# helemanc/audio-based-lyrics-matching

Hardware: NVIDIA B200
Metric: similarity+MAP eval Gpairs/s at 1/2/4/8 B200 (roofline frac); MAP parity (higher is better)
Workload: dtype f16 tensor-core hi/lo split x3, f32 accumulate

## Files before the change

audio-based-lyrics-matching_b200/csrc/eval_sym_epilogue.cuh:

```cuda
#pragma once
#include "gemm_core.cuh"

namespace wealy {

struct EvalSymParams {
  const float4* lvl;
  const uint2* cinfo;
  const int* s_c;
  const int* s_i;
  const float* thr;
  unsigned int* hist;
  const unsigned char* dirty;
  int n_col_tiles;
  int n_row_blocks;
  unsigned int total_pairs;
  const float* beta;
  float* tk_val;
  int* tk_idx;
  int* tk_cnt;
  int tk_cap;
};

__device__ __forceinline__ unsigned bit_transpose32(unsigned x, int lane) {
#pragma unroll
  for (int s = 16; s >= 1; s >>= 1) {
    const unsigned mask = s == 16 ? 0x0000ffffu : s == 8 ? 0x00ff00ffu : s == 4 ? 0x0f0f0f0fu : s == 2 ? 0x33333333u : 0x55555555u;
    const unsigned y = __shfl_xor_sync(0xffffffffu, x, s);
    x = (lane & s) ? ((x & ~mask) | ((y >> s) & mask)) : ((x & mask) | ((y << s) & ~mask));
  }
  return x;
}

template <int kLv, int kQueueCapT = 256, int kCachePairsT = 4096, bool kTopk = false>
struct EvalSymEpi {
  static_assert(kLv >= 2 && kLv <= 4, "2..4 register levels");
  static_assert(!kTopk || kLv <= 3, "the top-k bound of the columns rides in the 4th threshold slot");
  using Params = EvalSymParams;
  static constexpr int kQueueCap = kQueueCapT;
  static constexpr int kCachePairs = kCachePairsT;
  static constexpr unsigned kGlobal = 0x80000000u;
  static constexpr int kOffQx = kQueueCap * 4;
  static constexpr int kOffQn = kOffQx + kQueueCap * 4;
  static constexpr int kStageCols = 16;
  static constexpr int kOffStage = kOffQn + kQueueCap * 4;
  static constexpr int kWarpScratchBytes = kOffStage + kStageCols * 32 * 4;
  static constexpr int kColSlots = 3;
  static constexpr int kLvlBytes = kTileN * 16;
  static constexpr int kInfoBytes = kTileN * 8;
  static constexpr int kColSlotBytes = kLvlBytes + kInfoBytes;
  static constexpr int kOffColSlots = (kCachePairs * 4 + 15) / 16 * 16;
  static constexpr int kCtaScratchBytes = kOffColSlots + kColSlots * kColSlotBytes;

  __device__ static __forceinline__ void col_bulk_src(const Params& p, int t, const void*& s0, const void*& s1) {
    s0 = p.lvl + (size_t)t * kTileN;
    s1 = p.cinfo + (size_t)t * kTileN;
  }

  struct RowState {
    float t[kLv];
    unsigned rc[kLv - 1];
    unsigned rinfo;
    int rpc;
    int qc, qi;
    unsigned off;
    int qn;
    int n_cached;
    unsigned base;
    int row_glob, row_ok, dirty;
    float beta;
  };

  __device__ static __forceinline__ float* q_val(const EpiCtx& c) { return reinterpret_cast<float*>(c.warp_scratch); }
  __device__ static __forceinline__ unsigned* q_idx(const EpiCtx& c) { return reinterpret_cast<unsigned*>(c.warp_scratch + kOffQx); }
  __device__ static __forceinline__ int* q_len(const EpiCtx& c) { return reinterpret_cast<int*>(c.warp_scratch + kOffQn); }
  __device__ static __forceinline__ float* stage(const EpiCtx& c) { return reinterpret_cast<float*>(c.warp_scratch + kOffStage); }
  __device__ static __forceinline__ float* thr_s(const EpiCtx& c) { return reinterpret_cast<float*>(c.cta_scratch); }

  __device__ static __forceinline__ float lvl_of(const float4& v, int j) {
    return j == 0 ? v.x : (j == 1 ? v.y : (j == 2 ? v.z : v.w));
  }

  __device__ static __forceinline__ void row_begin(const Params& p, RowState& st, int row, int part,
                                                   const GemmShape& sh, const EpiCtx& ctx) {
    (void)part;
    const float inf = __int_as_float(0x7f800000);
#pragma unroll
    for (int j = 0; j < kLv; ++j) st.t[j] = inf;
#pragma unroll
    for (int j = 0; j < kLv - 1; ++j) st.rc[j] = 0u;
    st.qc = st.qi = 0;
    st.off = 0u;
    st.beta = inf;
    int cnt = 0;
    const int srow = spread_sorted_of(row);
    st.row_ok = srow < sh.m_rows;
    if (st.row_ok) {
      const float4 v = __ldg(p.lvl + row);
#pragma unroll
      for (int j = 0; j < kLv; ++j) st.t[j] = lvl_of(v, j);
      const uint2 ci = __ldg(p.cinfo + row);
      st.off = ci.x;
      cnt = (int)ci.y;
      st.qc = __ldg(p.s_c + srow);
      st.qi = __ldg(p.s_i + srow);
      if constexpr (kTopk) st.beta = __ldg(p.beta + row);
    }
    st.qn = 0;
    st.row_glob = row;
    st.dirty = 0;
    st.base = __ldg(p.cinfo + ctx.row_base).x;
    const unsigned end = (ctx.row_base + ctx.row_span < sh.m_rows) ? __ldg(p.cinfo + ctx.row_base + ctx.row_span).x : p.total_pairs;
    const unsigned total = end - st.base;
    st.n_cached = (int)(total < (unsigned)kCachePairs ? total : (unsigned)kCachePairs);
    float* ts = thr_s(ctx);
    for (int i = ctx.tid; i < st.n_cached; i += ctx.nthreads) ts[i] = __ldg(p.thr + st.base + i);
    const unsigned rel = st.off - st.base;
    const bool cached = st.row_ok && rel + (unsigned)cnt <= (unsigned)st.n_cached;
    st.rinfo = cached ? (rel + kLv) : (kGlobal | (st.off + kLv));
    st.rpc = cnt - kLv;
    ptx::named_barrier_sync(1, ctx.nthreads);
  }

  __device__ static __forceinline__ int warp_incl_scan(int v, int lane) {
#pragma unroll
    for (int o = 1; o < 32; o <<= 1) {
      const int t = __shfl_up_sync(0xffffffffu, v, o);
      if (lane >= o) v += t;
    }
    return v;
  }

  struct Ent {
    float s;
    unsigned idx;
    int len;
    int cand;
    bool on;
    const float* tp;
  };
  __device__ static __forceinline__ void fetch(const Params& p, const EpiCtx& ctx, Ent& en, int r, int end) {
    en.on = r < end;
    en.s = en.on ? q_val(ctx)[r] : 0.f;
    en.idx = en.on ? q_idx(ctx)[r] : 0u;
    const int raw = en.on ? q_len(ctx)[r] : 0;
    en.len = max(raw, 0);
    en.cand = kTopk ? -1 - raw : -1;
    en.tp = (en.idx & kGlobal) ? (p.thr + (en.idx & ~kGlobal)) : (thr_s(ctx) + en.idx);
  }
  __device__ static __forceinline__ void count(const Params& p, const RowState& st, const EpiCtx& ctx, const Ent& en,
                                               int lb, int lane) {
    (void)ctx; (void)lane;
    if constexpr (kTopk) {
      if (en.cand >= 0) {
        if (en.on) {
          const int pos = atomicAdd(p.tk_cnt + en.idx, 1);
          if (pos < p.tk_cap) {
            p.tk_val[(size_t)en.idx * p.tk_cap + pos] = en.s;
            p.tk_idx[(size_t)en.idx * p.tk_cap + pos] = en.cand;
          }
        }
        return;
      }
    }
    const bool glob = (en.idx & kGlobal) != 0u;
    const unsigned slot = (en.idx & ~kGlobal) - 1u + (unsigned)lb + (glob ? 0u : st.base);
    if (en.on) atomicAdd(p.hist + slot, 1u);
  }

  __device__ static __forceinline__ void drain(const Params& p, RowState& st, const EpiCtx& ctx) {
    if (st.qn == 0) return;
    const int lane = (int)ptx::lane_id();
    __syncwarp();
    const int end = st.qn;
    for (int r0 = 0; r0 < end; r0 += 64) {
      Ent a, b;
      fetch(p, ctx, a, r0 + lane, end);
      fetch(p, ctx, b, r0 + 32 + lane, end);
      int loa = 0, hia = a.len, lob = 0, hib = b.len;
      while (loa < hia || lob < hib) {
        if (loa < hia) {
          const int mid = (loa + hia) >> 1;
          if (a.tp[mid] < a.s) loa = mid + 1; else hia = mid;
        }
        if (lob < hib) {
          const int mid = (lob + hib) >> 1;
          if (b.tp[mid] < b.s) lob = mid + 1; else hib = mid;
        }
      }
      count(p, st, ctx, a, loa, lane);
      if (r0 + 32 < end) count(p, st, ctx, b, lob, lane);
    }
    __syncwarp();
    st.qn = 0;
  }

  __device__ static __forceinline__ void push(const RowState& st, const EpiCtx& ctx, const uint32_t (&acc)[32], unsigned mr,
                                              unsigned mcq, const uint2* cinf, int pos, unsigned tkr = 0u, unsigned tkc = 0u,
                                              int col0 = 0) {
    float* qv = q_val(ctx);
    unsigned* qx = q_idx(ctx);
    int* ql = q_len(ctx);
    float* stg = stage(ctx) + (ptx::lane_id());
#pragma unroll
    for (int h = 0; h < 32 / kStageCols; ++h) {
      const unsigned sel = ((1u << kStageCols) - 1u) << (h * kStageCols);
      if (!__any_sync(0xffffffffu, ((mr | mcq | tkr | tkc) & sel) != 0u)) continue;
#pragma unroll
      for (int e = 0; e < kStageCols; ++e) stg[e * 32] = __uint_as_float(acc[h * kStageCols + e]);
      unsigned m = mr & sel;
      while (m) {
        const int e = __ffs(m) - 1;
        m &= m - 1;
        qv[pos] = stg[(e - h * kStageCols) * 32];
        qx[pos] = st.rinfo;
        ql[pos] = st.rpc;
        ++pos;
      }
      m = mcq & sel;
      while (m) {
        const int e = __ffs(m) - 1;
        m &= m - 1;
        const uint2 c = cinf[e];
        qv[pos] = stg[(e - h * kStageCols) * 32];
        qx[pos] = kGlobal | (c.x + kLv);
        ql[pos] = (int)c.y - kLv;
        ++pos;
      }
      if constexpr (kTopk) {
        m = tkr & sel;
        while (m) {
          const int e = __ffs(m) - 1;
          m &= m - 1;
          qv[pos] = stg[(e - h * kStageCols) * 32];
          qx[pos] = (unsigned)st.row_glob;
          ql[pos] = -1 - (col0 + e);
          ++pos;
        }
        m = tkc & sel;
        while (m) {
          const int e = __ffs(m) - 1;
          m &= m - 1;
          qv[pos] = stg[(e - h * kStageCols) * 32];
          qx[pos] = (unsigned)(col0 + e);
          ql[pos] = -1 - st.row_glob;
          ++pos;
        }
      }
      __syncwarp();
    }
  }

  __device__ static __forceinline__ void tile_begin(const Params& p, RowState& st, const GemmShape& sh,
                                                    const EpiCtx& ctx, int t) {
    (void)sh;
    st.dirty = 0;
    for (int rbi = ctx.row_base / kTileM; rbi < (ctx.row_base + ctx.row_span) / kTileM; ++rbi)
      st.dirty |= rbi < p.n_row_blocks ? (int)__ldg(p.dirty + (size_t)rbi * p.n_col_tiles + t) : 1;
  }

  __device__ static __forceinline__ void chunk32(const Params& p, RowState& st, int row, int col0,
                                                 const uint32_t (&acc)[32], const GemmShape& sh, const EpiCtx& ctx) {
    constexpr unsigned kFull = 0xffffffffu;
    const int lane = (int)ptx::lane_id();
    (void)row;
    const float4* lv = reinterpret_cast<const float4*>(ctx.col_slot) + (col0 & (kTileN - 1));
    const uint2* cinf = reinterpret_cast<const uint2*>(ctx.col_slot + kLvlBytes) + (col0 & (kTileN - 1));

    unsigned m[kLv], mc[kLv];
    unsigned tkr = 0u, tkc = 0u;
#pragma unroll
    for (int j = 0; j < kLv; ++j) m[j] = mc[j] = 0u;
#pragma unroll
    for (int e = 0; e < 32; ++e) {
      const float s = __uint_as_float(acc[e]);
      const float4 c = lv[e];
#pragma unroll
      for (int j = 0; j < kLv; ++j) {
        m[j] |= (s > st.t[j]) ? (1u << e) : 0u;
        mc[j] |= (s > lvl_of(c, j)) ? (1u << e) : 0u;
      }
      if constexpr (kTopk) {
        tkr |= (s > st.beta) ? (1u << e) : 0u;
        tkc |= (s > c.w) ? (1u << e) : 0u;
      }
    }
    if (st.dirty) {
      const int scol = spread_sorted_of(col0 + lane);
      const bool ok = scol < sh.n_cols;
      const int cc = ok ? __ldg(p.s_c + scol) : 0;
      const int ci = ok ? __ldg(p.s_i + scol) : 0;
      unsigned valid = 0u, validk = 0u;
#pragma unroll
      for (int e = 0; e < 32; ++e) {
        const int cce = __shfl_sync(kFull, cc, e);
        const int cie = __shfl_sync(kFull, ci, e);
        const int oke = __shfl_sync(kFull, (int)ok, e);
        valid |= (oke && cce != st.qc && cie != st.qi) ? (1u << e) : 0u;
        if constexpr (kTopk) validk |= (oke && cie != st.qi) ? (1u << e) : 0u;
      }
      const int d = st.row_glob - col0;
      const unsigned above = d < 0 ? 0xffffffffu : (d >= 31 ? 0u : (0xffffffffu << (d + 1)));
      valid &= above;
      validk &= above;
      if (!st.row_ok) valid = validk = 0u;
#pragma unroll
      for (int j = 0; j < kLv; ++j) {
        m[j] &= valid;
        mc[j] &= valid;
      }
      tkr &= validk;
      tkc &= validk;
    }
    if constexpr (kTopk) {
      if (!__any_sync(kFull, (m[0] | mc[0] | tkr | tkc) != 0u)) return;
    } else {
      if (!__any_sync(kFull, (m[0] | mc[0]) != 0u)) return;
    }

#pragma unroll
    for (int j = 0; j < kLv - 1; ++j) st.rc[j] += (unsigned)__popc(m[j] ^ m[j + 1]);
    if (__any_sync(kFull, (mc[0] ^ mc[kLv - 1]) != 0u)) {
      const unsigned coff = cinf[lane].x;
#pragma unroll
      for (int j = 0; j < kLv - 1; ++j) {
        const unsigned n = (unsigned)__popc(bit_transpose32(mc[j] ^ mc[j + 1], lane));
        if (n != 0u) atomicAdd(p.hist + coff + j, n);
      }
    }

    const unsigned dr = m[kLv - 1], dc = mc[kLv - 1];
    if (!__any_sync(kFull, (dr | dc | tkr | tkc) != 0u)) return;
    const int mine = __popc(dr) + __popc(dc) + __popc(tkr) + __popc(tkc);
    const int incl = warp_incl_scan(mine, lane);
    const int total = __shfl_sync(kFull, incl, 31);
    if (st.qn + total > kQueueCap) drain(p, st, ctx);
    if (total <= kQueueCap) {
      push(st, ctx, acc, dr, dc, cinf, st.qn + incl - mine, tkr, tkc, col0);
      st.qn += total;
    } else {
      constexpr int kBatchCols = kQueueCap / (kTopk ? 128 : 64);
      static_assert(kBatchCols >= 1 && 32 % kBatchCols == 0, "queue capacity: 64 (128 with top-k) .. 2048, a power of two");
#pragma unroll 1
      for (int g = 0; g < 32 / kBatchCols; ++g) {
        const unsigned sel = ((1u << kBatchCols) - 1u) << (kBatchCols * g);
        const int mine_g = __popc(dr & sel) + __popc(dc & sel) + __popc(tkr & sel) + __popc(tkc & sel);
        const int incl_g = warp_incl_scan(mine_g, lane);
        push(st, ctx, acc, dr & sel, dc & sel, cinf, incl_g - mine_g, tkr & sel, tkc & sel, col0);
        st.qn = __shfl_sync(kFull, incl_g, 31);
        drain(p, st, ctx);
      }
    }
  }

  __device__ static __forceinline__ void tile_end(const Params& p, RowState& st, const GemmShape&, const EpiCtx& ctx) {
    if (st.qn >= kQueueCap / 2) drain(p, st, ctx);
  }

  __device__ static __forceinline__ void row_end(const Params& p, RowState& st, int row, int part,
                                                 const GemmShape& sh, const EpiCtx& ctx) {
    (void)row; (void)part; (void)sh;
    drain(p, st, ctx);
    if (st.row_ok) {
#pragma unroll
      for (int j = 0; j < kLv - 1; ++j)
        if (st.rc[j] != 0u) atomicAdd(p.hist + st.off + j, st.rc[j]);
    }
    ptx::named_barrier_sync(1, ctx.nthreads);
  }
};

}
```

audio-based-lyrics-matching_b200/csrc/ptx.cuh:

```cuda
#pragma once
#include <cstdint>
#include <cuda.h>
#include <cuda_runtime.h>

namespace wealy {
namespace ptx {

__device__ __forceinline__ uint32_t smem_u32(const void* p) {
  return static_cast<uint32_t>(__cvta_generic_to_shared(p));
}

__device__ __forceinline__ uint32_t lane_id() {
  uint32_t l;
  asm volatile("mov.u32 %0, %%laneid;" : "=r"(l));
  return l;
}

__device__ __forceinline__ void mbar_init(uint64_t* bar, uint32_t count) {
  asm volatile("mbarrier.init.shared::cta.b64 [%0], %1;" ::"r"(smem_u32(bar)), "r"(count));
}

__device__ __forceinline__ void fence_mbar_init() {
  asm volatile("fence.mbarrier_init.release.cluster;" ::: "memory");
}

__device__ __forceinline__ void fence_proxy_async() {
  asm volatile("fence.proxy.async.shared::cta;" ::: "memory");
}

__device__ __forceinline__ void mbar_expect_tx(uint64_t* bar, uint32_t bytes) {
  asm volatile("mbarrier.arrive.expect_tx.shared::cta.b64 _, [%0], %1;" ::"r"(smem_u32(bar)), "r"(bytes)
               : "memory");
}

__device__ __forceinline__ void mbar_arrive(uint64_t* bar) {
  asm volatile("mbarrier.arrive.shared::cta.b64 _, [%0];" ::"r"(smem_u32(bar)) : "memory");
}

#ifndef WEALY_WAIT_HINT_NS
#define WEALY_WAIT_HINT_NS 1000
#endif
#ifndef WEALY_WAIT_ALL_LANES
#define WEALY_WAIT_LANE0
#endif

__device__ __forceinline__ bool mbar_try_wait(uint64_t* bar, uint32_t parity) {
  uint32_t ok;
#if WEALY_WAIT_HINT_NS > 0
  asm volatile(
      "{\n"
      ".reg .pred P;\n"
      "mbarrier.try_wait.parity.shared::cta.b64 P, [%1], %2, %3;\n"
      "selp.u32 %0, 1, 0, P;\n"
      "}\n"
      : "=r"(ok)
      : "r"(smem_u32(bar)), "r"(parity), "r"((uint32_t)WEALY_WAIT_HINT_NS)
      : "memory");
#else
  asm volatile(
      "{\n"
      ".reg .pred P;\n"
      "mbarrier.try_wait.parity.shared::cta.b64 P, [%1], %2;\n"
      "selp.u32 %0, 1, 0, P;\n"
      "}\n"
      : "=r"(ok)
      : "r"(smem_u32(bar)), "r"(parity)
      : "memory");
#endif
  return ok != 0;
}

#ifndef WEALY_DEADLOCK_CYCLES
#define WEALY_DEADLOCK_CYCLES (4000000000ll)
#endif

__device__ __forceinline__ void mbar_wait(uint64_t* bar, uint32_t parity) {
  if (mbar_try_wait(bar, parity)) return;
  const long long t0 = clock64();
  int polls = 0;
  while (!mbar_try_wait(bar, parity)) {
    if ((++polls & 63) == 0 && clock64() - t0 > WEALY_DEADLOCK_CYCLES) {
      printf("wealy: mbarrier deadlock block=%d thread=%d bar=0x%x parity=%u\n", (int)blockIdx.x,
             (int)threadIdx.x, smem_u32(bar), parity);
      __trap();
    }
  }
}

__device__ __forceinline__ void mbar_wait_warp(uint64_t* bar, uint32_t parity) {
#ifdef WEALY_WAIT_LANE0
  if (lane_id() == 0) mbar_wait(bar, parity);
  __syncwarp();
#else
  mbar_wait(bar, parity);
#endif
}

__device__ __forceinline__ void named_barrier_sync(int id, int nthreads) {
  asm volatile("bar.sync %0, %1;" ::"r"(id), "r"(nthreads) : "memory");
}

__device__ __forceinline__ void prefetch_tensormap(const CUtensorMap* m) {
  asm volatile("prefetch.tensormap [%0];" ::"l"(reinterpret_cast<uint64_t>(m)) : "memory");
}

__device__ __forceinline__ void tma_load_2d(void* smem_dst, const CUtensorMap* m, uint64_t* bar, int32_t c0,
                                            int32_t c1, uint64_t cache_policy) {
  asm volatile(
      "cp.async.bulk.tensor.2d.shared::cluster.global.mbarrier::complete_tx::bytes.L2::cache_hint"
      " [%0], [%1, {%3, %4}], [%2], %5;"
      ::"r"(smem_u32(smem_dst)), "l"(reinterpret_cast<uint64_t>(m)), "r"(smem_u32(bar)), "r"(c0), "r"(c1),
        "l"(cache_policy)
      : "memory");
}

__device__ __forceinline__ void bulk_load(void* smem_dst, const void* gsrc, uint32_t bytes, uint64_t* bar) {
  asm volatile(
      "cp.async.bulk.shared::cluster.global.mbarrier::complete_tx::bytes [%0], [%1], %2, [%3];"
      ::"r"(smem_u32(smem_dst)), "l"(reinterpret_cast<uint64_t>(gsrc)), "r"(bytes), "r"(smem_u32(bar))
      : "memory");
}

constexpr uint64_t kEvictNormal = 0x1000000000000000ull;
constexpr uint64_t kEvictFirst = 0x12F0000000000000ull;
constexpr uint64_t kEvictLast = 0x14F0000000000000ull;

template <uint32_t kCols>
__device__ __forceinline__ void tmem_alloc(uint32_t* smem_result) {
  static_assert(kCols >= 32 && kCols <= 512 && (kCols & (kCols - 1)) == 0, "TMEM columns: power of two in [32,512]");
  asm volatile("tcgen05.alloc.cta_group::1.sync.aligned.shared::cta.b32 [%0], %1;" ::"r"(smem_u32(smem_result)),
               "n"(kCols)
               : "memory");
  asm volatile("tcgen05.relinquish_alloc_permit.cta_group::1.sync.aligned;" ::: "memory");
}

template <uint32_t kCols>
__device__ __forceinline__ void tmem_dealloc(uint32_t tmem_addr) {
  asm volatile("tcgen05.dealloc.cta_group::1.sync.aligned.b32 %0, %1;" ::"r"(tmem_addr), "n"(kCols) : "memory");
}

__device__ __forceinline__ void tc_fence_before_sync() {
  asm volatile("tcgen05.fence::before_thread_sync;" ::: "memory");
}
__device__ __forceinline__ void tc_fence_after_sync() {
  asm volatile("tcgen05.fence::after_thread_sync;" ::: "memory");
}

__device__ __forceinline__ void umma_f16(uint32_t tmem_d, uint64_t desc_a, uint64_t desc_b, uint32_t idesc,
                                         uint32_t accumulate) {
  asm volatile(
      "{\n"
      ".reg .pred p;\n"
      "setp.ne.b32 p, %4, 0;\n"
      "tcgen05.mma.cta_group::1.kind::f16 [%0], %1, %2, %3, p;\n"
      "}\n"
      ::"r"(tmem_d), "l"(desc_a), "l"(desc_b), "r"(idesc), "r"(accumulate)
      : "memory");
}

__device__ __forceinline__ void umma_commit(uint64_t* bar) {
  asm volatile("tcgen05.commit.cta_group::1.mbarrier::arrive::one.shared::cluster.b64 [%0];" ::"r"(smem_u32(bar))
               : "memory");
}

__device__ __forceinline__ void tmem_ld_32x32(uint32_t taddr, uint32_t (&v)[32]) {
  asm volatile(
      "tcgen05.ld.sync.aligned.32x32b.x32.b32 "
      "{%0, %1, %2, %3, %4, %5, %6, %7, %8, %9, %10, %11, %12, %13, %14, %15, "
      "%16, %17, %18, %19, %20, %21, %22, %23, %24, %25, %26, %27, %28, %29, %30, %31}, [%32];"
      : "=r"(v[0]), "=r"(v[1]), "=r"(v[2]), "=r"(v[3]), "=r"(v[4]), "=r"(v[5]), "=r"(v[6]), "=r"(v[7]), "=r"(v[8]),
        "=r"(v[9]), "=r"(v[10]), "=r"(v[11]), "=r"(v[12]), "=r"(v[13]), "=r"(v[14]), "=r"(v[15]), "=r"(v[16]),
        "=r"(v[17]), "=r"(v[18]), "=r"(v[19]), "=r"(v[20]), "=r"(v[21]), "=r"(v[22]), "=r"(v[23]), "=r"(v[24]),
        "=r"(v[25]), "=r"(v[26]), "=r"(v[27]), "=r"(v[28]), "=r"(v[29]), "=r"(v[30]), "=r"(v[31])
      : "r"(taddr)
      : "memory");
}

__device__ __forceinline__ void tmem_ld_wait() { asm volatile("tcgen05.wait::ld.sync.aligned;" ::: "memory"); }


__device__ __forceinline__ uint32_t cluster_ctarank() {
  uint32_t r;
  asm volatile("mov.u32 %0, %%cluster_ctarank;" : "=r"(r));
  return r;
}
__device__ __forceinline__ uint32_t cluster_id_x() {
  uint32_t r;
  asm volatile("mov.u32 %0, %%clusterid.x;" : "=r"(r));
  return r;
}
__device__ __forceinline__ uint32_t n_clusters_x() {
  uint32_t r;
  asm volatile("mov.u32 %0, %%nclusterid.x;" : "=r"(r));
  return r;
}
__device__ __forceinline__ void cluster_sync_all() {
  asm volatile("barrier.cluster.arrive.release.aligned;\n\tbarrier.cluster.wait.acquire.aligned;" ::: "memory");
}
__device__ __forceinline__ uint32_t map_to_cta(const void* p, uint32_t rank) {
  uint32_t r;
  asm volatile("mapa.shared::cluster.u32 %0, %1, %2;" : "=r"(r) : "r"(smem_u32(p)), "r"(rank));
  return r;
}
__device__ __forceinline__ void mbar_arrive_cluster(uint32_t cluster_addr) {
  asm volatile("mbarrier.arrive.release.cluster.shared::cluster.b64 _, [%0];" ::"r"(cluster_addr) : "memory");
}
__device__ __forceinline__ void mbar_arrive_cluster_relaxed(uint32_t cluster_addr) {
  asm volatile("mbarrier.arrive.relaxed.cluster.shared::cluster.b64 _, [%0];" ::"r"(cluster_addr) : "memory");
}
__device__ __forceinline__ void st_cluster_u32(uint32_t cluster_addr, uint32_t v) {
  asm volatile("st.shared::cluster.u32 [%0], %1;" ::"r"(cluster_addr), "r"(v) : "memory");
}
__device__ __forceinline__ void mbar_wait_cluster(uint64_t* bar, uint32_t parity) {
  const long long t0 = clock64();
  int polls = 0;
  while (true) {
    uint32_t ok;
    asm volatile(
        "{\n"
        ".reg .pred P;\n"
        "mbarrier.try_wait.parity.acquire.cluster.shared::cta.b64 P, [%1], %2, %3;\n"
        "selp.u32 %0, 1, 0, P;\n"
        "}\n"
        : "=r"(ok)
        : "r"(smem_u32(bar)), "r"(parity), "r"((uint32_t)(WEALY_WAIT_HINT_NS > 0 ? WEALY_WAIT_HINT_NS : 1))
        : "memory");
    if (ok) return;
    if ((++polls & 63) == 0 && clock64() - t0 > WEALY_DEADLOCK_CYCLES) {
      printf("wealy: cluster mbarrier deadlock block=%d thread=%d bar=0x%x parity=%u\n", (int)blockIdx.x,
             (int)threadIdx.x, smem_u32(bar), parity);
      __trap();
    }
  }
}

__device__ __forceinline__ void mbar_wait_cluster_warp(uint64_t* bar, uint32_t parity) {
  if (lane_id() == 0) mbar_wait_cluster(bar, parity);
  __syncwarp();
}

__device__ __forceinline__ void tma_load_2d_pair(void* smem_dst, const CUtensorMap* m, uint32_t leader_bar_addr, int32_t c0,
                                                 int32_t c1, uint64_t cache_policy) {
  asm volatile(
      "cp.async.bulk.tensor.2d.cta_group::2.shared::cluster.global.mbarrier::complete_tx::bytes.L2::cache_hint"
      " [%0], [%1, {%3, %4}], [%2], %5;"
      ::"r"(smem_u32(smem_dst)), "l"(reinterpret_cast<uint64_t>(m)), "r"(leader_bar_addr), "r"(c0), "r"(c1),
        "l"(cache_policy)
      : "memory");
}

template <uint32_t kCols>
__device__ __forceinline__ void tmem_alloc_pair(uint32_t* smem_result) {
  asm volatile("tcgen05.alloc.cta_group::2.sync.aligned.shared::cta.b32 [%0], %1;" ::"r"(smem_u32(smem_result)), "n"(kCols)
               : "memory");
  asm volatile("tcgen05.relinquish_alloc_permit.cta_group::2.sync.aligned;" ::: "memory");
}
template <uint32_t kCols>
__device__ __forceinline__ void tmem_dealloc_pair(uint32_t tmem_addr) {
  asm volatile("tcgen05.dealloc.cta_group::2.sync.aligned.b32 %0, %1;" ::"r"(tmem_addr), "n"(kCols) : "memory");
}

__device__ __forceinline__ void umma_f16_pair(uint32_t tmem_d, uint64_t desc_a, uint64_t desc_b, uint32_t idesc,
                                              uint32_t accumulate) {
  asm volatile(
      "{\n"
      ".reg .pred p;\n"
      "setp.ne.b32 p, %4, 0;\n"
      "tcgen05.mma.cta_group::2.kind::f16 [%0], %1, %2, %3, p;\n"
      "}\n"
      ::"r"(tmem_d), "l"(desc_a), "l"(desc_b), "r"(idesc), "r"(accumulate)
      : "memory");
}
__device__ __forceinline__ void umma_commit_pair(uint64_t* bar) {
  asm volatile(
      "tcgen05.commit.cta_group::2.mbarrier::arrive::one.shared::cluster.multicast::cluster.b64 [%0], %1;"
      ::"r"(smem_u32(bar)), "h"((uint16_t)3)
      : "memory");
}

template <int kSwizzleBytes>
__device__ __forceinline__ uint64_t make_smem_desc(uint32_t smem_addr) {
  static_assert(kSwizzleBytes == 128 || kSwizzleBytes == 64 || kSwizzleBytes == 32, "swizzle span");
  constexpr uint64_t layout = kSwizzleBytes == 128 ? 2ull : (kSwizzleBytes == 64 ? 4ull : 6ull);
  constexpr uint64_t sbo = (8ull * kSwizzleBytes) >> 4;
  return (uint64_t)((smem_addr & 0x3FFFFu) >> 4) | (1ull << 16) | (sbo << 32) | (1ull << 46) | (layout << 61);
}

__host__ __device__ constexpr uint32_t make_idesc_f16(int m, int n, bool bf16) {
  return (1u << 4) | ((bf16 ? 1u : 0u) << 7) | ((bf16 ? 1u : 0u) << 10) | ((uint32_t)(n >> 3) << 17) |
         ((uint32_t)(m >> 4) << 24);
}

}
}
```

Baseline: 428.8.

## Add counting fast path for clean tiles and cheapen deadlock polling clock

For tiles with no diagonal or same-clique masking (non-dirty, non-top-k), the epilogue now counts threshold crossings with set.gt float-to-1.0 sums decoded by a multiply trick, instead of building per-level bitmasks and popcounting them. Column counts come from transposing the accumulators through swizzled shared staging, so the per-level bit_transpose shuffles are no longer needed. The goal is fewer ALU and shuffle instructions in the hot epilogue. The price is shared-memory staging traffic and extra warp syncs. Separately, the mbarrier deadlock watchdog now reads clock64 only every 2048 polls and starts its timer lazily, which takes clock reads out of the spin loops.

```diff
diff --git a/audio-based-lyrics-matching_b200/csrc/eval_sym_epilogue.cuh b/audio-based-lyrics-matching_b200/csrc/eval_sym_epilogue.cuh
--- a/audio-based-lyrics-matching_b200/csrc/eval_sym_epilogue.cuh
+++ b/audio-based-lyrics-matching_b200/csrc/eval_sym_epilogue.cuh
@@ -258,77 +258,87 @@
       st.dirty |= rbi < p.n_row_blocks ? (int)__ldg(p.dirty + (size_t)rbi * p.n_col_tiles + t) : 1;
   }
 
-  __device__ static __forceinline__ void chunk32(const Params& p, RowState& st, int row, int col0,
-                                                 const uint32_t (&acc)[32], const GemmShape& sh, const EpiCtx& ctx) {
-    constexpr unsigned kFull = 0xffffffffu;
-    const int lane = (int)ptx::lane_id();
-    (void)row;
-    const float4* lv = reinterpret_cast<const float4*>(ctx.col_slot) + (col0 & (kTileN - 1));
-    const uint2* cinf = reinterpret_cast<const uint2*>(ctx.col_slot + kLvlBytes) + (col0 & (kTileN - 1));
-
-    unsigned m[kLv], mc[kLv];
-    unsigned tkr = 0u, tkc = 0u;
-#pragma unroll
-    for (int j = 0; j < kLv; ++j) m[j] = mc[j] = 0u;
+  __device__ static __forceinline__ unsigned gt_one(float a, float b) {
+    float r;
+    asm("set.gt.f32.f32 %0, %1, %2;" : "=f"(r) : "f"(a), "f"(b));
+    return __float_as_uint(r);
+  }
+  __device__ static __forceinline__ unsigned ones_count(unsigned sum) { return ((sum >> 23) * 383u) & 511u; }
+  __device__ static __forceinline__ void set_if_gt(unsigned& m, float a, float b, unsigned bit) {
+    asm("{\n.reg .pred p;\nsetp.gt.f32 p, %1, %2;\n@p or.b32 %0, %0, %3;\n}" : "+r"(m) : "f"(a), "f"(b), "r"(bit));
+  }
+
+  __device__ static __forceinline__ void chunk32_clean(const Params& p, RowState& st, int col0, const uint32_t (&acc)[32],
+                                                       const EpiCtx& ctx, const float4* lv, const uint2* cinf, int lane) {
+    constexpr int kCnt = kLv - 1;
+    unsigned nr[kCnt];
+    unsigned dr = 0u;
+#pragma unroll
+    for (int j = 0; j < kCnt; ++j) nr[j] = 0u;
 #pragma unroll
     for (int e = 0; e < 32; ++e) {
       const float s = __uint_as_float(acc[e]);
-      const float4 c = lv[e];
-#pragma unroll
-      for (int j = 0; j < kLv; ++j) {
-        m[j] |= (s > st.t[j]) ? (1u << e) : 0u;
-        mc[j] |= (s > lvl_of(c, j)) ? (1u << e) : 0u;
-      }
-      if constexpr (kTopk) {
-        tkr |= (s > st.beta) ? (1u << e) : 0u;
-        tkc |= (s > c.w) ? (1u << e) : 0u;
-      }
-    }
-    if (st.dirty) {
-      const int scol = spread_sorted_of(col0 + lane);
-      const bool ok = scol < sh.n_cols;
-      const int cc = ok ? __ldg(p.s_c + scol) : 0;
-      const int ci = ok ? __ldg(p.s_i + scol) : 0;
-      unsigned valid = 0u, validk = 0u;
-#pragma unroll
-      for (int e = 0; e < 32; ++e) {
-        const int cce = __shfl_sync(kFull, cc, e);
-        const int cie = __shfl_sync(kFull, ci, e);
-        const int oke = __shfl_sync(kFull, (int)ok, e);
-        valid |= (oke && cce != st.qc && cie != st.qi) ? (1u << e) : 0u;
-        if constexpr (kTopk) validk |= (oke && cie != st.qi) ? (1u << e) : 0u;
-      }
-      const int d = st.row_glob - col0;
-      const unsigned above = d < 0 ? 0xffffffffu : (d >= 31 ? 0u : (0xffffffffu << (d + 1)));
-      valid &= above;
-      validk &= above;
-      if (!st.row_ok) valid = validk = 0u;
-#pragma unroll
-      for (int j = 0; j < kLv; ++j) {
-        m[j] &= valid;
-        mc[j] &= valid;
-      }
-      tkr &= validk;
-      tkc &= validk;
-    }
-    if constexpr (kTopk) {
-      if (!__any_sync(kFull, (m[0] | mc[0] | tkr | tkc) != 0u)) return;
-    } else {
-      if (!__any_sync(kFull, (m[0] | mc[0]) != 0u)) return;
-    }
-
-#pragma unroll
-    for (int j = 0; j < kLv - 1; ++j) st.rc[j] += (unsigned)__popc(m[j] ^ m[j + 1]);
-    if (__any_sync(kFull, (mc[0] ^ mc[kLv - 1]) != 0u)) {
+#pragma unroll
+      for (int j = 0; j < kCnt; ++j) nr[j] += gt_one(s, st.t[j]);
+      set_if_gt(dr, s, st.t[kCnt], 1u << e);
+    }
+#pragma unroll
+    for (int j = 0; j < kCnt - 1; ++j) st.rc[j] += ones_count(nr[j] - nr[j + 1]);
+    st.rc[kCnt - 1] += ones_count(nr[kCnt - 1]) - (unsigned)__popc(dr);
+
+    float* stg = stage(ctx);
+    const int cc = lane & 15, r0 = lane & 16;
+    unsigned cpk = 0u, cdm = 0u;
+#pragma unroll
+    for (int h = 0; h < 2; ++h) {
+#pragma unroll
+      for (int e = 0; e < 16; ++e) stg[e * 32 + (lane ^ ((e & 7) << 2))] = __uint_as_float(acc[h * 16 + e]);
+      __syncwarp();
+      const float4 tc = lv[h * 16 + cc];
+      const float* src = stg + cc * 32;
+      const int sw = (cc & 7) << 2;
+      unsigned nc[kCnt];
+      unsigned dch = 0u;
+#pragma unroll
+      for (int j = 0; j < kCnt; ++j) nc[j] = 0u;
+#pragma unroll
+      for (int k = 0; k < 4; ++k) {
+        const float4 q = *reinterpret_cast<const float4*>(src + ((r0 + 4 * k) ^ sw));
+        const float v4[4] = {q.x, q.y, q.z, q.w};
+#pragma unroll
+        for (int i = 0; i < 4; ++i) {
+#pragma unroll
+          for (int j = 0; j < kCnt; ++j) nc[j] += gt_one(v4[i], lvl_of(tc, j));
+          set_if_gt(dch, v4[i], lvl_of(tc, kCnt), 1u << (4 * k + i));
+        }
+      }
+      __syncwarp();
+      unsigned pk = (ones_count(nc[kCnt - 1]) - (unsigned)__popc(dch)) << (8 * (kCnt - 1));
+#pragma unroll
+      for (int j = 0; j < kCnt - 1; ++j) pk += ones_count(nc[j] - nc[j + 1]) << (8 * j);
+      pk += __shfl_xor_sync(0xffffffffu, pk, 16);
+      const unsigned other = __shfl_xor_sync(0xffffffffu, dch, 16);
+      if ((lane >> 4) == h) {
+        cpk = pk;
+        cdm = r0 ? (other | (dch << 16)) : (dch | (other << 16));
+      }
+    }
+    if (cpk != 0u) {
       const unsigned coff = cinf[lane].x;
 #pragma unroll
-      for (int j = 0; j < kLv - 1; ++j) {
-        const unsigned n = (unsigned)__popc(bit_transpose32(mc[j] ^ mc[j + 1], lane));
+      for (int j = 0; j < kCnt; ++j) {
+        const unsigned n = (cpk >> (8 * j)) & 0xffu;
         if (n != 0u) atomicAdd(p.hist + coff + j, n);
       }
     }
-
-    const unsigned dr = m[kLv - 1], dc = mc[kLv - 1];
+    const unsigned dc = __any_sync(0xffffffffu, cdm != 0u) ? bit_transpose32(cdm, lane) : 0u;
+    enqueue(p, st, ctx, acc, dr, dc, 0u, 0u, cinf, col0, lane);
+  }
+
+  __device__ static __forceinline__ void enqueue(const Params& p, RowState& st, const EpiCtx& ctx, const uint32_t (&acc)[32],
+                                                 unsigned dr, unsigned dc, unsigned tkr, unsigned tkc, const uint2* cinf,
+                                                 int col0, int lane) {
+    constexpr unsigned kFull = 0xffffffffu;
     if (!__any_sync(kFull, (dr | dc | tkr | tkc) != 0u)) return;
     const int mine = __popc(dr) + __popc(dc) + __popc(tkr) + __popc(tkc);
     const int incl = warp_incl_scan(mine, lane);
@@ -352,6 +362,85 @@
     }
   }
 
+  __device__ static __forceinline__ void chunk32(const Params& p, RowState& st, int row, int col0,
+                                                 const uint32_t (&acc)[32], const GemmShape& sh, const EpiCtx& ctx) {
+    constexpr unsigned kFull = 0xffffffffu;
+    const int lane = (int)ptx::lane_id();
+    (void)row;
+    const float4* lv = reinterpret_cast<const float4*>(ctx.col_slot) + (col0 & (kTileN - 1));
+    const uint2* cinf = reinterpret_cast<const uint2*>(ctx.col_slot + kLvlBytes) + (col0 & (kTileN - 1));
+    if constexpr (!kTopk) {
+      if (!st.dirty) {
+        chunk32_clean(p, st, col0, acc, ctx, lv, cinf, lane);
+        return;
+      }
+    }
+
+    unsigned m[kLv], mc[kLv];
+    unsigned tkr = 0u, tkc = 0u;
+#pragma unroll
+    for (int j = 0; j < kLv; ++j) m[j] = mc[j] = 0u;
+#pragma unroll
+    for (int e = 0; e < 32; ++e) {
+      const float s = __uint_as_float(acc[e]);
+      const float4 c = lv[e];
+#pragma unroll
+      for (int j = 0; j < kLv; ++j) {
+        m[j] |= (s > st.t[j]) ? (1u << e) : 0u;
+        mc[j] |= (s > lvl_of(c, j)) ? (1u << e) : 0u;
+      }
+      if constexpr (kTopk) {
+        tkr |= (s > st.beta) ? (1u << e) : 0u;
+        tkc |= (s > c.w) ? (1u << e) : 0u;
+      }
+    }
+    if (st.dirty) {
+      const int scol = spread_sorted_of(col0 + lane);
+      const bool ok = scol < sh.n_cols;
+      const int cc = ok ? __ldg(p.s_c + scol) : 0;
+      const int ci = ok ? __ldg(p.s_i + scol) : 0;
+      unsigned valid = 0u, validk = 0u;
+#pragma unroll
+      for (int e = 0; e < 32; ++e) {
+        const int cce = __shfl_sync(kFull, cc, e);
+        const int cie = __shfl_sync(kFull, ci, e);
+        const int oke = __shfl_sync(kFull, (int)ok, e);
+        valid |= (oke && cce != st.qc && cie != st.qi) ? (1u << e) : 0u;
+        if constexpr (kTopk) validk |= (oke && cie != st.qi) ? (1u << e) : 0u;
+      }
+      const int d = st.row_glob - col0;
+      const unsigned above = d < 0 ? 0xffffffffu : (d >= 31 ? 0u : (0xffffffffu << (d + 1)));
+      valid &= above;
+      validk &= above;
+      if (!st.row_ok) valid = validk = 0u;
+#pragma unroll
+      for (int j = 0; j < kLv; ++j) {
+        m[j] &= valid;
+        mc[j] &= valid;
+      }
+      tkr &= validk;
+      tkc &= validk;
+    }
+    if constexpr (kTopk) {
+      if (!__any_sync(kFull, (m[0] | mc[0] | tkr | tkc) != 0u)) return;
+    } else {
+      if (!__any_sync(kFull, (m[0] | mc[0]) != 0u)) return;
+    }
+
+#pragma unroll
+    for (int j = 0; j < kLv - 1; ++j) st.rc[j] += (unsigned)__popc(m[j] ^ m[j + 1]);
+    if (__any_sync(kFull, (mc[0] ^ mc[kLv - 1]) != 0u)) {
+      const unsigned coff = cinf[lane].x;
+#pragma unroll
+      for (int j = 0; j < kLv - 1; ++j) {
+        const unsigned n = (unsigned)__popc(bit_transpose32(mc[j] ^ mc[j + 1], lane));
+        if (n != 0u) atomicAdd(p.hist + coff + j, n);
+      }
+    }
+
+    enqueue(p, st, ctx, acc, m[kLv - 1], mc[kLv - 1], tkr, tkc, cinf, col0, lane);
+  }
+
   __device__ static __forceinline__ void tile_end(const Params& p, RowState& st, const GemmShape&, const EpiCtx& ctx) {
     if (st.qn >= kQueueCap / 2) drain(p, st, ctx);
   }
diff --git a/audio-based-lyrics-matching_b200/csrc/ptx.cuh b/audio-based-lyrics-matching_b200/csrc/ptx.cuh
--- a/audio-based-lyrics-matching_b200/csrc/ptx.cuh
+++ b/audio-based-lyrics-matching_b200/csrc/ptx.cuh
@@ -74,17 +74,28 @@
 #define WEALY_DEADLOCK_CYCLES (4000000000ll)
 #endif
 
-__device__ __forceinline__ void mbar_wait(uint64_t* bar, uint32_t parity) {
-  if (mbar_try_wait(bar, parity)) return;
-  const long long t0 = clock64();
+constexpr int kClockPolls = 2048;
+struct DeadlockClock {
+  long long t0 = 0;
   int polls = 0;
-  while (!mbar_try_wait(bar, parity)) {
-    if ((++polls & 63) == 0 && clock64() - t0 > WEALY_DEADLOCK_CYCLES) {
-      printf("wealy: mbarrier deadlock block=%d thread=%d bar=0x%x parity=%u\n", (int)blockIdx.x,
-             (int)threadIdx.x, smem_u32(bar), parity);
+  __device__ __forceinline__ void tick(const char* what, uint64_t* bar, uint32_t parity) {
+    if (++polls < kClockPolls) return;
+    polls = 0;
+    const long long now = clock64();
+    if (t0 == 0) {
+      t0 = now;
+    } else if (now - t0 > WEALY_DEADLOCK_CYCLES) {
+      printf("wealy: %s deadlock block=%d thread=%d bar=0x%x parity=%u\n", what, (int)blockIdx.x, (int)threadIdx.x,
+             smem_u32(bar), parity);
       __trap();
     }
   }
+};
+
+__device__ __forceinline__ void mbar_wait(uint64_t* bar, uint32_t parity) {
+  if (mbar_try_wait(bar, parity)) return;
+  DeadlockClock clk;
+  while (!mbar_try_wait(bar, parity)) clk.tick("mbarrier", bar, parity);
 }
 
 __device__ __forceinline__ void mbar_wait_warp(uint64_t* bar, uint32_t parity) {
@@ -211,27 +222,24 @@
 __device__ __forceinline__ void st_cluster_u32(uint32_t cluster_addr, uint32_t v) {
   asm volatile("st.shared::cluster.u32 [%0], %1;" ::"r"(cluster_addr), "r"(v) : "memory");
 }
+__device__ __forceinline__ bool mbar_try_wait_cluster(uint64_t* bar, uint32_t parity) {
+  uint32_t ok;
+  asm volatile(
+      "{\n"
+      ".reg .pred P;\n"
+      "mbarrier.try_wait.parity.acquire.cluster.shared::cta.b64 P, [%1], %2, %3;\n"
+      "selp.u32 %0, 1, 0, P;\n"
+      "}\n"
+      : "=r"(ok)
+      : "r"(smem_u32(bar)), "r"(parity), "r"((uint32_t)(WEALY_WAIT_HINT_NS > 0 ? WEALY_WAIT_HINT_NS : 1))
+      : "memory");
+  return ok != 0;
+}
+
 __device__ __forceinline__ void mbar_wait_cluster(uint64_t* bar, uint32_t parity) {
-  const long long t0 = clock64();
-  int polls = 0;
-  while (true) {
-    uint32_t ok;
-    asm volatile(
-        "{\n"
-        ".reg .pred P;\n"
-        "mbarrier.try_wait.parity.acquire.cluster.shared::cta.b64 P, [%1], %2, %3;\n"
-        "selp.u32 %0, 1, 0, P;\n"
-        "}\n"
-        : "=r"(ok)
-        : "r"(smem_u32(bar)), "r"(parity), "r"((uint32_t)(WEALY_WAIT_HINT_NS > 0 ? WEALY_WAIT_HINT_NS : 1))
-        : "memory");
-    if (ok) return;
-    if ((++polls & 63) == 0 && clock64() - t0 > WEALY_DEADLOCK_CYCLES) {
-      printf("wealy: cluster mbarrier deadlock block=%d thread=%d bar=0x%x parity=%u\n", (int)blockIdx.x,
-             (int)threadIdx.x, smem_u32(bar), parity);
-      __trap();
-    }
-  }
+  if (mbar_try_wait_cluster(bar, parity)) return;
+  DeadlockClock clk;
+  while (!mbar_try_wait_cluster(bar, parity)) clk.tick("cluster mbarrier", bar, parity);
 }
 
 __device__ __forceinline__ void mbar_wait_cluster_warp(uint64_t* bar, uint32_t parity) {
```

After: 443.1 (median of 6 runs). 1.03x the previous value.
